# sunwj/SunVolumeRender

Hardware: AMD Instinct MI355X
Metric: Msamples/sec (paths x spp) at 1024^2 on 512^3 volume (higher is better)
Workload: dtype f32; 1 GPU; c3: 512^3 u16 CT-like volume, 1024x1024 image, 3 area lights, env map on, trace depth 1, 256 spp per step; math=bit-exact contract, parallelism=single GPU

## Files before the change

### include/svr_abi.h

```cpp
#ifndef SVR_ABI_H
#define SVR_ABI_H

#include <stddef.h>
#include <stdint.h>

#ifdef __cplusplus
extern "C" {
#endif

#define SVR_MAX_LIGHT_SOURCES 8
#define SVR_TF_TABLE_SIZE 1024

typedef struct svr_vec2 { float x, y; } svr_vec2;
typedef struct svr_vec3 { float x, y, z; } svr_vec3;

typedef struct svr_bbox {
    svr_vec3 vmin, vmax, invSize;
} svr_bbox;

typedef struct svr_volume {
    svr_bbox bbox;
    uint32_t _pad0;
    uint64_t tex;
    float densityScale;
// ... 147 lines not shown
    uint64_t vol_taps;
    uint64_t woodcock_iters;
    uint64_t scatter_events;
    uint64_t shadow_walks;
    uint64_t raycast_steps;
    uint64_t loop_iters;
    uint64_t vol_taps_executed;
    uint64_t walks_ray_skipped;
    uint64_t iters_ray_skipped;
    uint64_t iters_prefix_skipped;
    uint64_t taps_bound_culled;
} svr_counters;
int svr_selftest_chain(const float* items, float* results, uint32_t n);
int svr_selftest_math(int fn, const float* in, uint32_t in_stride, float* out, uint32_t n);
int svr_selftest_bound8(const float* rays, uint32_t n, uint32_t* out);
int svr_macro_grid(int nx, int ny, int nz, int shift_min, int out[8]);
int svr_selftest_accel(int table, void* out, size_t out_bytes, int32_t info[16]);
typedef struct svr_denoise_params {
    int32_t passes;
    float sigma_depth;
    float sigma_normal;
    float sigma_albedo;
    float sigma_opacity;
    float sigma_color;
    float step;
} svr_denoise_params;
int svr_denoise_params_default(svr_denoise_params* p);
int svr_set_denoise_params(const svr_denoise_params* p);
int svr_get_denoise_params(svr_denoise_params* p);
int svr_render_guides(void* guides);
// ... 239 lines not shown
```

### sunvolumerender_amd/abi.py

```python
from __future__ import annotations

import ctypes as C
from pathlib import Path

from ._build import LIB_PATH



class vec2(C.Structure):
    _fields_ = [("x", C.c_float), ("y", C.c_float)]

    def __init__(self, x=0.0, y=0.0):
        super().__init__(float(x), float(y))

    def tuple(self):
        return (self.x, self.y)


class vec3(C.Structure):
    _fields_ = [("x", C.c_float), ("y", C.c_float), ("z", C.c_float)]

    def __init__(self, x=0.0, y=0.0, z=0.0):
        super().__init__(float(x), float(y), float(z))

# ... 313 lines not shown
OPT_LOCAL_MAJORANT = 23
OPT_LIGHT_CULL = 24
OPT_LM_TUNE = 25
OPT_LM_SUBCELLS = 26
OPT_PARK_CHEAP = 27
OPT_PINHOLE_FAST = 28
OPT_POOL = 29
OPT_TRIPS = 30
OPT_NAN_GUARD = 31
OPT_MACRO_SHIFT_MIN = 32
OPT_SPLIT = 33
OPT_ENV_NEE = 34
OPT_FAST_BOUND = 35
OPT_DENOISE_PREVIEW = 36
OPT_NOISE_ESTIMATE = 37
KERNEL_AUTO, KERNEL_PIXEL, KERNEL_TILE, KERNEL_ULOOP, KERNEL_WAVEFRONT = 0, 1, 2, 3, 4

ELEM_I8, ELEM_U8, ELEM_I16, ELEM_U16, ELEM_I32, ELEM_U32, ELEM_F32, ELEM_F64 = range(8)


class MhdHeader(C.Structure):
    _fields_ = [
        ("ndims", C.c_int32), ("dim", C.c_int32 * 3), ("spacing", C.c_double * 3),
        ("elem_type", C.c_int32), ("elem_size", C.c_int32), ("channels", C.c_int32), ("msb", C.c_int32),
        ("compressed", C.c_int32), ("compressed_size", C.c_int64), ("header_size", C.c_int64),
        ("data_offset", C.c_int64), ("data_file", C.c_char * 1024),
    ]


class VolumeInfo(C.Structure):
# ... 35 lines not shown
    "svr_strip_rows_owned": (C.c_uint32, [C.c_uint32, C.c_uint32, C.c_uint32, C.c_uint32]),
    "svr_strip_row_to_y": (C.c_uint32, [C.c_uint32, C.c_uint32, C.c_uint32, C.c_uint32, C.c_uint32]),
    "svr_pack_strips": (C.c_int, [C.c_void_p, C.c_void_p, C.c_uint32, C.c_uint32, C.c_uint32, C.c_uint32, C.c_uint32]),
    "svr_unpack_strips": (C.c_int, [C.c_void_p, C.c_void_p, C.c_uint32, C.c_uint32, C.c_uint32, C.c_uint32, C.c_uint32]),
    "svr_assemble_frame": (C.c_int, [C.c_void_p, C.c_void_p, C.c_void_p, C.c_uint32, C.c_uint32, C.c_uint32, C.c_uint32, C.c_uint32, C.c_uint32]),
    "svr_set_row_shard": (C.c_int, [C.c_uint32, C.c_uint32, C.c_uint32]),
    "svr_set_render_window": (C.c_int, [C.c_int, C.c_int, C.c_int, C.c_int]),
    "svr_set_option": (C.c_int, [C.c_int, C.c_int]),
    "svr_get_option": (C.c_int, [C.c_int]),
    "svr_render_pathtracer_frames": (C.c_int, [C.c_void_p, _P(RenderParams), C.c_uint32]),
    "svr_hdr_to_ldr": (C.c_int, [C.c_void_p, _P(RenderParams)]),
    "svr_hdr_to_ldr_frame": (C.c_int, [C.c_void_p, C.c_void_p, C.c_uint32, C.c_uint32]),
    "svr_selftest_chain": (C.c_int, [C.c_void_p, C.c_void_p, C.c_uint32]),
    "svr_selftest_math": (C.c_int, [C.c_int, C.c_void_p, C.c_uint32, C.c_void_p, C.c_uint32]),
    "svr_selftest_bound8": (C.c_int, [C.c_void_p, C.c_uint32, C.c_void_p]),
    "svr_macro_grid": (C.c_int, [C.c_int, C.c_int, C.c_int, C.c_int, _P(C.c_int)]),
    "svr_selftest_accel": (C.c_int, [C.c_int, C.c_void_p, C.c_size_t, _P(C.c_int32)]),
    "svr_denoise_params_default": (C.c_int, [_P(DenoiseParams)]),
    "svr_set_denoise_params": (C.c_int, [_P(DenoiseParams)]),
    "svr_get_denoise_params": (C.c_int, [_P(DenoiseParams)]),
    "svr_render_guides": (C.c_int, [C.c_void_p]),
    "svr_denoise_to_ldr": (C.c_int, [C.c_void_p, C.c_void_p, C.c_uint32, C.c_uint32, _P(DenoiseParams)]),
    "svr_denoise_hdr": (C.c_int, [C.c_void_p, C.c_void_p, C.c_uint32, C.c_uint32, _P(DenoiseParams)]),
    "svr_guide_builds": (C.c_uint64, []),
    "svr_get_noise_estimate": (C.c_int, [_P(NoiseEstimate), C.c_void_p]),
    "svr_estimate_noise": (C.c_int, [C.c_void_p, C.c_uint32, C.c_void_p, C.c_uint32, C.c_uint32, C.c_uint32, C.c_void_p, _P(NoiseEstimate)]),
    "svr_render_pathtracer_until": (C.c_int, [C.c_void_p, _P(RenderParams), C.c_float, C.c_float, C.c_uint32, _P(C.c_uint32)]),
    "svr_render_pathtracer_adaptive": (C.c_int, [C.c_void_p, _P(RenderParams), C.c_float, C.c_uint32, C.c_uint32, _P(AdaptiveResult)]),
    "svr_get_adaptive_tiles": (C.c_int, [C.c_void_p, C.c_void_p]),
    "svr_projection_params_default": (C.c_int, [_P(ProjectionParams)]),
# ... 101 lines not shown
```

### sunvolumerender_amd/csrc/svr_api.hip

```cpp
#include "../../include/svr_abi.h"
#include "svr_kernels.hpp"
#include "svr_denoise.hpp"
#include "svr_noise.hpp"
#include "svr_project.hpp"
#include "svr_slice.hpp"
#include "svr_hits.hpp"
#include "svr_device.hpp"

#include <hip/hip_runtime.h>
#include <algorithm>
#include <cmath>
#include <cstdarg>
#include <cstdio>
#include <cstdlib>
#include <cstring>
#include <dlfcn.h>
#include <mutex>
#include <string>
#include <unordered_map>
#include <vector>

static_assert(sizeof(svr_vec3) == 12, "glm::vec3 layout");
static_assert(sizeof(svr_bbox) == 36, "cudaBBox layout");
static_assert(sizeof(svr_volume) == 112 && offsetof(svr_volume, tex) == 40 && offsetof(svr_volume, densityScale) == 48 &&
// ... 2401 lines not shown
    case SVR_OPT_QUEUE: return g.opt_queue;
    case SVR_OPT_PARK_END: return g.opt_park_end;
    case SVR_OPT_PARK_CHEAP: return g.opt_park_cheap;
    case SVR_OPT_PINHOLE_FAST: return g.opt_pinhole_fast;
    case SVR_OPT_POOL: return g.opt_pool;
    case SVR_OPT_TRIPS: return g.opt_trips;
    case SVR_OPT_SPLIT: return g.opt_split;
    case SVR_OPT_ENV_NEE: return g.opt_env_nee;
    case SVR_OPT_FAST_BOUND: return g.opt_fast_bound;
    case SVR_OPT_NAN_GUARD: return g.opt_nan_guard;
    case SVR_OPT_MACRO_SHIFT_MIN: return g.opt_macro_shift_min;
    case SVR_OPT_REFILL_MIN_IDLE: return g.opt_refill;
    case SVR_OPT_FRAMES_PER_WAVE_LOG2: return g.opt_frames_log2;
    case SVR_OPT_RAYCAST_LANES_LOG2: return g.opt_rc_lanes;
    case SVR_OPT_FRAME_AHEAD: return g.opt_frame_ahead;
    default: return -1;
    }
}

int svr_selftest_chain(const float* items, float* results, uint32_t n)
{
    if (ensure_init()) return g.err_code;
    if (!items || !results || n == 0) return fail(-4, "svr_selftest_chain: bad arguments");
    float4* d_buf = nullptr;
    HIP_TRY(hipMalloc((void**)&d_buf, (size_t)n * 32));
    hipError_t e = hipMemcpy(d_buf, items, (size_t)n * 16, hipMemcpyHostToDevice);
    if (e == hipSuccess) e = svr::launch_chain_selftest(d_buf, d_buf + n, n, g.stream);
    if (e == hipSuccess) e = hipStreamSynchronize(g.stream);
    if (e == hipSuccess) e = hipMemcpy(results, d_buf + n, (size_t)n * 16, hipMemcpyDeviceToHost);
    hipFree(d_buf);
// ... 25 lines not shown
    if (!g.have_vol || !g.have_tf || !g.have_cam) return fail(-4, "svr_selftest_bound8 before setup_volume/setup_transferfunction/setup_camera");
    svr::DevScene s;
    if (build_scene(g.vol, g.tf, g.cam, s)) return g.err_code;
    if (ensure_mask(s, g.vol, g.tf)) return g.err_code;
    if (s.bnd8 == nullptr) return fail(-3, "svr_selftest_bound8: the fast bound look-up is not in use for this scene");
    float* d_rays = nullptr; uint32_t* d_out = nullptr;
    HIP_TRY(hipMalloc((void**)&d_rays, (size_t)n * 7 * sizeof(float)));
    hipError_t e = hipMalloc((void**)&d_out, (size_t)n * sizeof(uint32_t));
    if (e == hipSuccess) e = hipMemcpy(d_rays, rays, (size_t)n * 7 * sizeof(float), hipMemcpyHostToDevice);
    if (e == hipSuccess) e = svr::launch_bound8_selftest(s, d_rays, n, d_out, g.stream);
    if (e == hipSuccess) e = hipStreamSynchronize(g.stream);
    if (e == hipSuccess) e = hipMemcpy(out, d_out, (size_t)n * sizeof(uint32_t), hipMemcpyDeviceToHost);
    hipFree(d_rays);
    if (d_out) hipFree(d_out);
    if (e != hipSuccess) return fail((int)e, "svr_selftest_bound8 failed: %s", hipGetErrorName(e));
    return 0;
}

int svr_selftest_accel(int table, void* out, size_t out_bytes, int32_t info[16])
{
    if (ensure_init()) return g.err_code;
    if (!info || table < 0 || table > 7 || (table != 0 && !out)) return fail(-4, "svr_selftest_accel: bad arguments");
    if (!g.have_vol || !g.have_tf || !g.have_cam) return fail(-4, "svr_selftest_accel before setup_volume/setup_transferfunction/setup_camera");
    svr::DevScene s;
    if (build_scene(g.vol, g.tf, g.cam, s)) return g.err_code;
    if (ensure_mask(s, g.vol, g.tf)) return g.err_code;
    const Texture* tv = find_tex(g.vol.tex, TEX_VOLUME);
    if (s.empty_mask == nullptr || !tv) return fail(-3, "svr_selftest_accel: the scene has no acceleration data (SVR_OPT_EMPTY_SKIP off?)");
    const int hgx = (tv->mc_gx + 1) / 2, hgy = (tv->mc_gy + 1) / 2, hgz = (tv->mc_gz + 1) / 2;
    const size_t n = (size_t)tv->mc_gx * tv->mc_gy * tv->mc_gz, hn = (size_t)hgx * hgy * hgz;
// ... 71 lines not shown
```

### sunvolumerender_amd/csrc/svr_kernels.hpp

```cpp
#pragma once
#include <hip/hip_runtime.h>
#include <type_traits>
#include "svr_scene.hpp"

namespace svr {

enum { KERNEL_AUTO = 0, KERNEL_PIXEL = 1, KERNEL_TILE = 2, KERNEL_ULOOP = 3, KERNEL_WAVEFRONT = 4, KERNEL_ENV_NEE = 5  };
constexpr int WF_QUEUE_PLANES = 18;
constexpr uint32_t TICKET_SHARDS = 8;
constexpr uint32_t TICKET_STRIDE = 32;
constexpr uint32_t MASK_WORDS_MAX = 8192;
constexpr uint32_t DIST_WORDS_MAX = 4096;
constexpr int DIST_CAP = 15;
constexpr uint32_t REC_C1_WORDS = 17;
constexpr uint32_t REC_A_WORDS = 26;
constexpr uint32_t REC_B_WORDS = 20;
constexpr uint32_t REC_WORDS = REC_A_WORDS + REC_B_WORDS;
constexpr uint32_t QUEUE_TASKS = 32;
constexpr uint32_t QUEUE_CAP = 32 * QUEUE_TASKS;
#ifndef SVR_QUEUE_TASKS_D1
#define SVR_QUEUE_TASKS_D1 64
#endif
#ifndef SVR_QUEUE_CAP_D1
#define SVR_QUEUE_CAP_D1 1024
// ... 72 lines not shown
hipError_t launch_fine_mask(const uint16_t* mm, uint32_t n_cells, const uint32_t* tf_zero_prefix, int tf_n, float densityScale,
                            uint32_t* mask, uint32_t words, hipStream_t stream);
hipError_t launch_sub8(const uint32_t* fine_empty, int fgx, int fgy, int fgz, int gx, int gy, int gz, uint8_t* sub8, hipStream_t stream);
hipError_t launch_bound_class(const uint16_t* mm, int gx, int gy, int gz, const float* tf_rgba, int tf_n, float densityScale,
                              float invSigmaMax, uint32_t* accel, hipStream_t stream);
constexpr uint32_t BOUND8_DIM = 34u;
constexpr uint32_t BOUND8_BYTES = 40960u;
hipError_t launch_bound8(const uint16_t* mm_wide, int hgx, int hgy, int hgz, const float* tf_rgba, int tf_n, float densityScale,
                         float invSigmaMax, uint8_t* bnd8, hipStream_t stream);
hipError_t launch_strips(float* packed, float* frame, uint32_t row_floats, uint32_t n_rows, uint32_t strip_rows, uint32_t rank, uint32_t world,
                         int to_packed, hipStream_t stream);
hipError_t launch_tonemap(const DevScene& scene, const DevWork& work, hipStream_t stream);
hipError_t launch_chain_selftest(const float4* in, float4* out, uint32_t n, hipStream_t stream);
hipError_t launch_math_selftest(int fn, const float* in, uint32_t in_stride, float* out, uint32_t n, hipStream_t stream);
hipError_t launch_bound8_selftest(const DevScene& scene, const float* rays, uint32_t n, uint32_t* out, hipStream_t stream);
hipError_t launch_raycast(const DevScene& scene, const DevWork& work, float stepSize, bool count, int num_cus, int lanes_log2, hipStream_t stream);
hipError_t launch_repack(const uint16_t* src, uint16_t* dst, int nx, int ny, int nz, int layout,
                         int sy, int sz, int bnx, int bny, hipStream_t stream);

}
```

### sunvolumerender_amd/csrc/svr_lanes.hpp

```cpp
#pragma once
#include "svr_walk.hpp"
#include "svr_tile_tasks.hpp"

namespace svr {


enum { PH_PRIMARY = 0, PH_REFILL, PH_SHADE, PH_CHEAP, PH_FETCH, PH_MARCH, PH_END, PH_FOLD, PH_N };
enum { PH_TICKET = PH_N + 1, PH_LOOP, PH_FIRST, PH_END_ALL };
enum { PROF_SHADOW_WALKS = 2 * PH_END_ALL, PROF_RECORDS };
constexpr uint32_t PROF_WORDS = 2 * PH_END_ALL + 2;
#ifdef SVR_TEST_HOOKS
#define SVR_PROF 1
struct ProfScope {
    unsigned long long* acc; uint32_t ph; uint64_t t0;
    __device__ ProfScope(unsigned long long* a, uint32_t p) : acc(a), ph(p), t0(__builtin_amdgcn_s_memtime()) {}
    __device__ void end(uint32_t lanes)
    {
        const uint64_t dt = __builtin_amdgcn_s_memtime() - t0;
        if ((threadIdx.x & 63u) == 0u) { atomicAdd(&acc[2 * ph], (unsigned long long)dt); atomicAdd(&acc[2 * ph + 1], (unsigned long long)dt * lanes); }
    }
};
#define PROF_BEGIN(name, ph) ProfScope name(c_prof, ph)
#define PROF_END(name, lanes) name.end(lanes)
#else
#define SVR_PROF 0
// ... 647 lines not shown
```

### sunvolumerender_amd/csrc/svr_primary.hpp

```cpp
#pragma once
#include "svr_walk.hpp"
#include "svr_lanes.hpp"

namespace svr {

#ifndef SVR_SHADOW_REMARCH
#define SVR_SHADOW_REMARCH true
#endif
#ifndef SVR_PRIMARY_REMARCH
#define SVR_PRIMARY_REMARCH false
#endif

template <int LAYOUT, bool COUNT, bool SKIP, typename LDS>
SVR_DEV bool trace_primary(const DevScene& s, const LDS& L_, uint32_t x, uint32_t y, uint32_t hashed, bool group_march, uint32_t P2,
                           GroupMapShared* gslot, Cnt& c, Rng& rng, v3& L, v3& pt, v3& wo, float& val, const DevScene* scp = nullptr)
{
    const DevScene& sc = scp ? *scp : s;
    uint32_t offset = y * sc.imageW + x;
    rng_init(rng, hashed + offset);
    if (COUNT) c.paths++;
    L = V3(0.f, 0.f, 0.f);
    const v3 T = V3(1.f, 1.f, 1.f);
    v3 orig, dir;
    camera_ray(sc, x, y, rng, orig, dir);
    float ls_t;
    int ls_id = nearest_light(sc, orig, dir, ls_t);
    float tMin = (float)1e-6, tMax = SVR_FLT_MAX;
    val = 0.f;
    float t;
    if (SKIP && group_march) {
        float t_occ;
        GroupMap map;
        map.g = gslot + ((threadIdx.x & 63u) & ((1u << P2) - 1u) & (GROUP_MAPS_PER_WAVE - 1u));
        int r = walk_setup_group<COUNT, SKIP>(s, L_, P2, orig, dir, false, tMin, tMax, t_occ, map);
        t = r <= 0 ? -SVR_FLT_MAX
                   : walk_run<LAYOUT, COUNT, SKIP, false, true>(s, L_, orig, dir, rng, tMin, tMax, t_occ, val, false, c, &map, P2);
    } else
        t = walk<LAYOUT, COUNT, SKIP, SVR_PRIMARY_REMARCH>(s, L_, orig, dir, rng, tMin, tMax, val, false, c);
    if (ls_id >= 0) {
        float tt = t < 0.f ? SVR_FLT_MAX : t;
        if (ls_t < tt) {
            const DevLight& l = sc.lights[ls_id];
            float cosTerm = dot(V3(l.normal[0], l.normal[1], l.normal[2]), -dir);
            L = L + (T * V3(l.radiance[0], l.radiance[1], l.radiance[2])) * (cosTerm <= 0.f ? 0.f : 1.f);
            return false;
        }
    }
    if (t < 0.f) {
        if (sc.env_on_escape) L = L + T * env_radiance(sc, dir);
// ... 40 lines not shown
```

### sunvolumerender_amd/csrc/svr_selftest.hip

```cpp
#include "svr_kernels.hpp"
#include "svr_device.hpp"
#include "svr_walk.hpp"
#include "svr_chain.hpp"

namespace svr {

__global__ __launch_bounds__(256) void k_math_selftest(int fn, const float* __restrict__ in, uint32_t stride, float* __restrict__ out, uint32_t n)
{
    const uint32_t i = blockIdx.x * 256u + threadIdx.x;
    if (i >= n) return;
    const float* a = in + (size_t)i * stride;
    const float x = a[0], y = stride > 1 ? a[1] : 0.f, z = stride > 2 ? a[2] : 0.f;
    float r = 0.f, sn, cs;
    switch (fn) {
    case 0: r = schlick_fresnel(x, y, z); break;
    case 1: r = logf_(x); break;
    case 2: r = expf_(x); break;
    case 3: sincosf_(x, &sn, &cs); r = sn; break;
    case 4: sincosf_(x, &sn, &cs); r = cs; break;
    case 5: r = acosf_(x); break;
    case 6: r = atan2f_(x, y); break;
    case 7: r = powf_(x, y); break;
    case 8: {
        Rng g;
// ... 43 lines not shown
}

hipError_t launch_bound8_selftest(const DevScene& s, const float* rays, uint32_t n, uint32_t* out, hipStream_t st)
{
    const dim3 grid((n + 255u) / 256u), block(256);
    switch (s.layout) {
    case 1: hipLaunchKernelGGL(k_bound8_selftest<1>, grid, block, 0, st, s, rays, n, out); break;
    case 2: hipLaunchKernelGGL(k_bound8_selftest<2>, grid, block, 0, st, s, rays, n, out); break;
    case 3: hipLaunchKernelGGL(k_bound8_selftest<3>, grid, block, 0, st, s, rays, n, out); break;
    case 4: hipLaunchKernelGGL(k_bound8_selftest<4>, grid, block, 0, st, s, rays, n, out); break;
    default: return hipErrorInvalidValue;
    }
    return hipGetLastError();
}

__global__ void k_chain_selftest(const float4* __restrict__ in, float4* __restrict__ out, uint32_t n_items)
{
    uint32_t i = blockIdx.x * blockDim.x + threadIdx.x;
    if (i >= n_items) return;
    const float4 q = in[i];
    bool e0, e1, ok;
    const uint32_t c0 = chain_count(q.x, q.y, q.z, false, e0);
    const uint32_t c1 = chain_count(q.x, q.y, q.z, true, e1);
    const float ta = chain_advance(q.x, q.y, (uint32_t)q.w, ok);
    out[i] = make_float4(__uint_as_float(c0), __uint_as_float(c1), ta, __uint_as_float((e0 ? 1u : 0u) | (e1 ? 2u : 0u) | (ok ? 4u : 0u)));
}

hipError_t launch_chain_selftest(const float4* in, float4* out, uint32_t n, hipStream_t st)
{
    hipLaunchKernelGGL(k_chain_selftest, dim3((n + 255u) / 256u), dim3(256), 0, st, in, out, n);
// ... 5 lines not shown
```

### sunvolumerender_amd/csrc/svr_trace_tile.hip

```cpp
#include "svr_walk.hpp"
#include "svr_lanes.hpp"
#include "svr_tile_tasks.hpp"
#include "svr_primary.hpp"

namespace svr {

#ifdef SVR_TEST_HOOKS
#define SVR_DEBUG_STOPS 1
#else
#define SVR_DEBUG_STOPS 0
#endif

#ifndef SVR_SHADOW_REMARCH
#define SVR_SHADOW_REMARCH true
#endif
#ifndef SVR_PRIMARY_REMARCH
#define SVR_PRIMARY_REMARCH false
#endif

template <int LAYOUT, bool COUNT, bool SKIP, bool DEPTH1, typename LDS>
SVR_DEV v3 trace_path_tile(const DevScene& s, const LDS& L_, uint32_t x, uint32_t y, uint32_t traceDepth_,
                           uint32_t hashed, uint32_t debug_stop, bool group_march, uint32_t P2, GroupMapShared* gslot, Cnt& c)
{
    const uint32_t traceDepth = DEPTH1 ? 1u : traceDepth_;
// ... 144 lines not shown
    const uint32_t wave = threadIdx.x >> 6;
#ifndef SVR_COLD_SCENE
#define SVR_COLD_SCENE 1
#endif
    auto cold_scene = [&]() -> const DevScene* {
        if constexpr (QUEUE && (DEPTH1 || (POOL && SVR_COLD_DEEP_POOL) || SVR_COLD_DEEP_ALL) && SVR_COLD_SCENE) {
            auto p = __builtin_amdgcn_kernarg_segment_ptr();
            asm volatile("" : "+s"(p));
            return (const DevScene*)p;
        } else return nullptr;
    };
    const TaskShape ts = task_shape(w);
    const uint32_t fl2 = ts.fl2, P2 = ts.P2, tw2 = ts.tw2, th2 = ts.th2, wv = ts.wv, fgroups = ts.fgroups;
    const uint32_t n_tasks = ts.n_tasks;
    Cnt c = {0, 0, 0, 0, 0, 0, 0, 0, 0, 0};

    const uint32_t unit = w.unit;
    const uint32_t n_units = (n_tasks + unit - 1u) / unit;
    const uint32_t shard0 = blockIdx.x % TICKET_SHARDS;
    const bool fold = w.fold != 0u;
    uint32_t npend = 0, qC = 0, qA = 0, qB = 0;
    LaneQueue Q;
    Q.cap = DRAIN_CAP;
    Q.q = QUEUE ? w.queue + (size_t)(blockIdx.x * TILE_WAVES + wave) * (REC_WORDS * DRAIN_CAP) : nullptr;
    float* const gpend = QUEUE ? w.pend + (size_t)(blockIdx.x * TILE_WAVES + wave) * (DRAIN_TASKS * 3u * 64u) : nullptr;
    auto flush = [&]() {
        if constexpr (QUEUE) {
            __builtin_amdgcn_fence(__ATOMIC_RELEASE, "workgroup");
            __builtin_amdgcn_fence(__ATOMIC_ACQUIRE, "workgroup");
            if constexpr (POOL && !DEPTH1) {
// ... 128 lines not shown
                    Rng rng = {0u, 0u, 0u, 0u, 0u, 0u};
                    v3 L = V3(0.f, 0.f, 0.f);
                    bool hit = false;
                    float val = 0.f;
                    Shade vs;
                    vs.pt = L; vs.wo = L; vs.gradient = L; vs.color[0] = vs.color[1] = vs.color[2] = vs.color[3] = 0.f; vs.Pbrdf = 0.f; vs.st = 0;
                    Nee ne;
                    ne.wi = L; ne.B = L; ne.pdf = 1.f; ne.light = 0u; ne.have = false;
#if SVR_PROF
                    unsigned long long* c_prof = w.counters + CNT_N;
#endif
                    PROF_BEGIN(pa, PH_PRIMARY);
#if SVR_PROF
                    const uint32_t prof_i0 = c.iters - c.iskip;
#endif
                    if (live) {
                        uint32_t x = w.x0 + px, y = owned_row_to_y(w, r);
                        hit = trace_primary<LAYOUT, COUNT, SKIP>(s, lds, x, y, wang_hash(w.frame0 + slot), group_march, P2, &gmaps[wave][0], c, rng, L, vs.pt, vs.wo, val, cold_scene());
                    }
                    PROF_END(pa, (uint32_t)__popcll(__ballot(live)));
#if SVR_PROF
                    if (COUNT && DEPTH1) {
                        const uint32_t d = (c.iters - c.iskip) - prof_i0;
                        uint32_t m = d;
                        for (int o = 32; o > 0; o >>= 1) m = max(m, (uint32_t)__shfl_xor((int)m, o));
                        const unsigned long long sum = wave_sum(d);
                        if (lane == 0) { atomicAdd(&c_prof[2 * PH_N], (unsigned long long)m * 64ull); atomicAdd(&c_prof[2 * PH_N + 1], sum); }
                    }
#endif
                    const bool shade_here = DEPTH1 || !s.bound_cull;
                    {
                        const uint64_t mh = __ballot(hit);
                        if (shade_here && mh != 0ull) {
                            PROF_BEGIN(psh, PH_SHADE);
// ... 99 lines not shown
    PROF_END(ploop, 64u);
    if (COUNT) cnt_flush(w, c);
}

template <int LAYOUT, bool COUNT>
static hipError_t launch_tile_t(const DevScene& s, const DevWork& w, const LaunchCfg& cfg, hipStream_t st)
{
    uint32_t wv = w.x1 - w.x0;
    if (wv == 0 || w.n_rows == 0) return hipSuccess;
    if (w.fold && w.nframes > 64u) return hipErrorInvalidValue;
    DevWork w2;
    TaskGrid g;
    hipError_t e = task_launch_setup(w, cfg, SVR_TILE_THREADS / 64, w.fold != 0u, cfg.frames_log2, st, w2, g);
    if (e != hipSuccess) return e;
    const uint32_t blocks = g.blocks;
    if (cfg.unit_override > 0) w2.unit = (uint32_t)cfg.unit_override;
    const bool skip = s.empty_mask != nullptr, d1 = w.traceDepth == 1u;
    const bool queue = LAYOUT != LAYOUT_LINEAR && w.queue != nullptr && w.pend != nullptr && blocks <= w.queue_blocks && w.traceDepth < 32768u &&
                       (w.fold || !COUNT);
#define SVR_LAUNCH_TILE(SK, D1, QU) hipLaunchKernelGGL((k_trace_tile<LAYOUT, COUNT, SK, D1, QU>), dim3(blocks), dim3(SVR_TILE_THREADS), 0, st, s, w2)
    if constexpr (LAYOUT != LAYOUT_LINEAR && !COUNT) {
        if (queue && !w.fold) {
#define SVR_LAUNCH_DIRECT(SK, D1, PO) hipLaunchKernelGGL((k_trace_tile<LAYOUT, false, SK, D1, true, PO, true>), dim3(blocks), dim3(SVR_TILE_THREADS), 0, st, s, w2)
            if (skip && cfg.pool_primary) { if (d1) SVR_LAUNCH_DIRECT(true, true, true); else SVR_LAUNCH_DIRECT(true, false, true); }
            else if (skip && d1) SVR_LAUNCH_DIRECT(true, true, false);
            else if (skip) SVR_LAUNCH_DIRECT(true, false, false);
            else if (d1) SVR_LAUNCH_DIRECT(false, true, false);
            else SVR_LAUNCH_DIRECT(false, false, false);
#undef SVR_LAUNCH_DIRECT
            return hipGetLastError();
        }
    }
    if constexpr (LAYOUT != LAYOUT_LINEAR) {
        if (queue && skip && cfg.pool_primary) {
// ... 29 lines not shown
```

### sunvolumerender_amd/csrc/svr_walk.hpp

```cpp
#pragma once
#include "svr_kernel_common.hpp"
#include <type_traits>

namespace svr {

struct LdsTile {
    float alpha[SVR_TF_MAX + SVR_TF_PAD];
    uint32_t dist[DIST_WORDS_MAX];
    uint32_t mask[MASK_WORDS_MAX];
    uint32_t emask[MASK_WORDS_MAX];
};
struct LdsTileNoMask {
    float alpha[SVR_TF_MAX + SVR_TF_PAD];
    uint32_t dist[1];
    uint32_t mask[1];
    uint32_t emask[1];
};
struct LdsTileCull : LdsTile {
    uint32_t cls[DIST_WORDS_MAX];
    float thr[BOUND_CLASSES];
};
struct LdsBound8 {
    uint8_t bnd[BOUND8_BYTES];
};
// ... 244 lines not shown
    struct { float lo, dt, inv_dt; const uint64_t* w; } g = {gm.lo, gm.dt, gm.inv_dt, gm.g->w};
    const uint32_t fl2 = 6u - P2, Lg = 64u >> P2;
    int ki = (int)((t - g.lo) * g.inv_dt) - 1;
    const uint32_t k = (uint32_t)(ki < 0 ? 0 : ki);
    const uint32_t r = k >> fl2, j = k & (Lg - 1u);
    uint64_t w0 = r == 0u ? g.w[0] : (r == 1u ? g.w[1] : (r == 2u ? g.w[2] : 0ull));
    w0 >>= (j << P2);
    if (w0) return fma_((float)(k + ((uint32_t)__builtin_ctzll(w0) >> P2)), g.dt, g.lo);
    const uint64_t w1 = r == 0u ? g.w[1] : (r == 1u ? g.w[2] : 0ull);
    if (w1) return fma_((float)(((r + 1u) << fl2) + ((uint32_t)__builtin_ctzll(w1) >> P2)), g.dt, g.lo);
    const uint64_t w2 = r == 0u ? g.w[2] : 0ull;
    if (w2) return fma_((float)(((r + 2u) << fl2) + ((uint32_t)__builtin_ctzll(w2) >> P2)), g.dt, g.lo);
    return u2f(SVR_INF_BITS);
}

template <typename LDS>
SVR_DEV float first_occupied_group(const DevScene& s, const LDS& L, uint32_t P2, v3 o, v3 d, bool hit, float tMin, float tMax, bool& ok,
                                   GroupMap& map)
{
    GroupMapShared& ms = *map.g;
    map.valid = false; map.lo = 0.f; map.dt = 1.f; map.inv_dt = 1.f;
    for (uint32_t r = 0; r < GROUP_MAP_ROUNDS; ++r) ms.w[r] = 0ull;
    const float INF = u2f(SVR_INF_BITS);
    const uint32_t lane = threadIdx.x & 63u;
    const uint32_t pl = lane & ((1u << P2) - 1u), m = lane >> P2, Lg = 64u >> P2;
    const int leader = (int)pl;
    const v3 oc = V3(__shfl(o.x, leader, 64), __shfl(o.y, leader, 64), __shfl(o.z, leader, 64));
    const v3 dc = V3(__shfl(d.x, leader, 64), __shfl(d.y, leader, 64), __shfl(d.z, leader, 64));
    float lo = hit ? tMin : INF, hi = hit ? tMax : -INF;
    for (uint32_t off = 32u; off >= (1u << P2); off >>= 1) {
// ... 24 lines not shown
        const int iz = min(max((int)__builtin_floorf(fma_(Bz, tk, Az)), 0), gz - 1);
        const uint32_t q = (uint32_t)(ix + iy * gx + iz * s.mc_gxy);
        const bool occupied = (tk <= hi) && !((L.mask[q >> 5] >> (q & 31u)) & 1u);
        const uint64_t b = __ballot(occupied) & gmask;
        if (round < GROUP_MAP_ROUNDS) ms.w[round] = b >> pl;
        if (b && !found) { found = true; result = fma_((float)(k0 + (((uint32_t)__builtin_ctzll(b) - pl) >> P2)), dt, lo); }
        const bool at_end = fma_((float)(k0 + Lg - 1u), dt, lo) > hi;
        if (at_end) { complete = round < GROUP_MAP_ROUNDS; break; }
        if (found && round + 1u >= GROUP_MAP_ROUNDS) break;
    }
    map.lo = lo; map.dt = dt; map.inv_dt = bmax * (1.f / 0.7f);
    map.valid = complete && ok;
    __builtin_amdgcn_fence(__ATOMIC_RELEASE, "wavefront");
    __builtin_amdgcn_fence(__ATOMIC_ACQUIRE, "wavefront");
    return result;
}

template <bool COUNT, bool SKIP, typename LDS>
SVR_DEV int walk_setup(const DevScene& s, const LDS& L, v3 orig, v3 dir, bool rng_live, float& tMin, float& tMax, float& t_occ)
{
    float tNear, tFar;
    if (!volume_intersect(s, orig, dir, tNear, tFar)) return -1;
    tMin = tNear < 0.f ? (float)1e-6 : tNear;
    tMax = tFar;
    t_occ = tMin;
    if (SKIP && s.ray_skip) {
        t_occ = first_occupied(s, L, orig, dir, tMin, tMax);
        if (!COUNT && !rng_live && t_occ == u2f(SVR_INF_BITS)) return 0;
    }
    return 1;
// ... 134 lines not shown
```

Baseline: 10720 Msamples/s.

## Share wave-wide empty-space march across 2x1 pixel blocks for pinhole primaries

Adds a shared group march for pinhole primary rays. A wave marches the macro-cell occupancy grid once along a central ray and keeps the result in LDS, tagged by a 2x1 pixel block and frame group. A later wave-step on the same block reuses it when every lane's ray passes an admission test (same origin, small angular deviation, interval contained). The launch sets the work unit to the march block size so consecutive tasks hit the same block. The aim is to halve the occupancy-grid marching cost per primary ray. Rays that fail admission fall back to a per-ray first_occupied walk, and there is added LDS state and branching. A selftest entry point is also added.

```diff
diff --git a/include/svr_abi.h b/include/svr_abi.h
--- a/include/svr_abi.h
+++ b/include/svr_abi.h
@@ -185,6 +185,7 @@
 int svr_selftest_chain(const float* items, float* results, uint32_t n);
 int svr_selftest_math(int fn, const float* in, uint32_t in_stride, float* out, uint32_t n);
 int svr_selftest_bound8(const float* rays, uint32_t n, uint32_t* out);
+int svr_selftest_group_march(uint32_t frame0, uint64_t out[8]);
 int svr_macro_grid(int nx, int ny, int nz, int shift_min, int out[8]);
 int svr_selftest_accel(int table, void* out, size_t out_bytes, int32_t info[16]);
 typedef struct svr_denoise_params {
diff --git a/sunvolumerender_amd/abi.py b/sunvolumerender_amd/abi.py
--- a/sunvolumerender_amd/abi.py
+++ b/sunvolumerender_amd/abi.py
@@ -351,6 +351,7 @@
 OPT_FAST_BOUND = 35
 OPT_DENOISE_PREVIEW = 36
 OPT_NOISE_ESTIMATE = 37
+OPT_UNIT = 101
 KERNEL_AUTO, KERNEL_PIXEL, KERNEL_TILE, KERNEL_ULOOP, KERNEL_WAVEFRONT = 0, 1, 2, 3, 4
 
 ELEM_I8, ELEM_U8, ELEM_I16, ELEM_U16, ELEM_I32, ELEM_U32, ELEM_F32, ELEM_F64 = range(8)
@@ -416,6 +417,7 @@
     "svr_selftest_chain": (C.c_int, [C.c_void_p, C.c_void_p, C.c_uint32]),
     "svr_selftest_math": (C.c_int, [C.c_int, C.c_void_p, C.c_uint32, C.c_void_p, C.c_uint32]),
     "svr_selftest_bound8": (C.c_int, [C.c_void_p, C.c_uint32, C.c_void_p]),
+    "svr_selftest_group_march": (C.c_int, [C.c_uint32, C.c_void_p]),
     "svr_macro_grid": (C.c_int, [C.c_int, C.c_int, C.c_int, C.c_int, _P(C.c_int)]),
     "svr_selftest_accel": (C.c_int, [C.c_int, C.c_void_p, C.c_size_t, _P(C.c_int32)]),
     "svr_denoise_params_default": (C.c_int, [_P(DenoiseParams)]),
diff --git a/sunvolumerender_amd/csrc/svr_api.hip b/sunvolumerender_amd/csrc/svr_api.hip
--- a/sunvolumerender_amd/csrc/svr_api.hip
+++ b/sunvolumerender_amd/csrc/svr_api.hip
@@ -2439,6 +2439,7 @@
     case SVR_OPT_FRAMES_PER_WAVE_LOG2: return g.opt_frames_log2;
     case SVR_OPT_RAYCAST_LANES_LOG2: return g.opt_rc_lanes;
     case SVR_OPT_FRAME_AHEAD: return g.opt_frame_ahead;
+    case 101: return g.opt_unit;
     default: return -1;
     }
 }
@@ -2494,6 +2495,26 @@
     hipFree(d_rays);
     if (d_out) hipFree(d_out);
     if (e != hipSuccess) return fail((int)e, "svr_selftest_bound8 failed: %s", hipGetErrorName(e));
+    return 0;
+}
+
+int svr_selftest_group_march(uint32_t frame0, uint64_t out[8])
+{
+    if (ensure_init()) return g.err_code;
+    if (!out) return fail(-4, "svr_selftest_group_march: bad arguments");
+    if (!g.have_vol || !g.have_tf || !g.have_cam) return fail(-4, "svr_selftest_group_march before setup_volume/setup_transferfunction/setup_camera");
+    svr::DevScene s;
+    if (build_scene(g.vol, g.tf, g.cam, s)) return g.err_code;
+    if (ensure_mask(s, g.vol, g.tf)) return g.err_code;
+    if (s.empty_mask == nullptr || !s.ray_skip) return fail(-3, "svr_selftest_group_march: the scene has no whole-ray test (SVR_OPT_EMPTY_SKIP off, or a clip box beyond the volume)");
+    unsigned long long* d_out = nullptr;
+    HIP_TRY(hipMalloc((void**)&d_out, 8 * sizeof(unsigned long long)));
+    hipError_t e = hipMemsetAsync(d_out, 0, 8 * sizeof(unsigned long long), g.stream);
+    if (e == hipSuccess) e = svr::launch_group_march_selftest(s, frame0, d_out, g.stream);
+    if (e == hipSuccess) e = hipStreamSynchronize(g.stream);
+    if (e == hipSuccess) e = hipMemcpy(out, d_out, 8 * sizeof(unsigned long long), hipMemcpyDeviceToHost);
+    hipFree(d_out);
+    if (e != hipSuccess) return fail((int)e, "svr_selftest_group_march failed: %s", hipGetErrorName(e));
     return 0;
 }
 
diff --git a/sunvolumerender_amd/csrc/svr_kernels.hpp b/sunvolumerender_amd/csrc/svr_kernels.hpp
--- a/sunvolumerender_amd/csrc/svr_kernels.hpp
+++ b/sunvolumerender_amd/csrc/svr_kernels.hpp
@@ -110,6 +110,7 @@
 hipError_t launch_chain_selftest(const float4* in, float4* out, uint32_t n, hipStream_t stream);
 hipError_t launch_math_selftest(int fn, const float* in, uint32_t in_stride, float* out, uint32_t n, hipStream_t stream);
 hipError_t launch_bound8_selftest(const DevScene& scene, const float* rays, uint32_t n, uint32_t* out, hipStream_t stream);
+hipError_t launch_group_march_selftest(const DevScene& scene, uint32_t frame0, unsigned long long* out, hipStream_t stream);
 hipError_t launch_raycast(const DevScene& scene, const DevWork& work, float stepSize, bool count, int num_cus, int lanes_log2, hipStream_t stream);
 hipError_t launch_repack(const uint16_t* src, uint16_t* dst, int nx, int ny, int nz, int layout,
                          int sy, int sz, int bnx, int bny, hipStream_t stream);
diff --git a/sunvolumerender_amd/csrc/svr_lanes.hpp b/sunvolumerender_amd/csrc/svr_lanes.hpp
--- a/sunvolumerender_amd/csrc/svr_lanes.hpp
+++ b/sunvolumerender_amd/csrc/svr_lanes.hpp
@@ -7,8 +7,9 @@
 
 enum { PH_PRIMARY = 0, PH_REFILL, PH_SHADE, PH_CHEAP, PH_FETCH, PH_MARCH, PH_END, PH_FOLD, PH_N };
 enum { PH_TICKET = PH_N + 1, PH_LOOP, PH_FIRST, PH_END_ALL };
-enum { PROF_SHADOW_WALKS = 2 * PH_END_ALL, PROF_RECORDS };
-constexpr uint32_t PROF_WORDS = 2 * PH_END_ALL + 2;
+enum { PROF_SHADOW_WALKS = 2 * PH_END_ALL, PROF_RECORDS, PROF_MARCH };
+constexpr uint32_t PROF_WORDS = 2 * PH_END_ALL + 6;
+static_assert(PROF_WORDS <= 32u, "the debug words behind the counters (svr_api.hip, DEBUG_WORDS)");
 #ifdef SVR_TEST_HOOKS
 #define SVR_PROF 1
 struct ProfScope {
diff --git a/sunvolumerender_amd/csrc/svr_primary.hpp b/sunvolumerender_amd/csrc/svr_primary.hpp
--- a/sunvolumerender_amd/csrc/svr_primary.hpp
+++ b/sunvolumerender_amd/csrc/svr_primary.hpp
@@ -11,9 +11,10 @@
 #define SVR_PRIMARY_REMARCH false
 #endif
 
-template <int LAYOUT, bool COUNT, bool SKIP, typename LDS>
+template <int LAYOUT, bool COUNT, bool SKIP, bool SHARE = false, typename LDS>
 SVR_DEV bool trace_primary(const DevScene& s, const LDS& L_, uint32_t x, uint32_t y, uint32_t hashed, bool group_march, uint32_t P2,
-                           GroupMapShared* gslot, Cnt& c, Rng& rng, v3& L, v3& pt, v3& wo, float& val, const DevScene* scp = nullptr)
+                           GroupMapShared* gslot, Cnt& c, Rng& rng, v3& L, v3& pt, v3& wo, float& val, const DevScene* scp = nullptr, uint32_t fg = 0u,
+                           uint32_t* march_did = nullptr)
 {
     const DevScene& sc = scp ? *scp : s;
     uint32_t offset = y * sc.imageW + x;
@@ -32,7 +33,13 @@
         float t_occ;
         GroupMap map;
         map.g = gslot + ((threadIdx.x & 63u) & ((1u << P2) - 1u) & (GROUP_MAPS_PER_WAVE - 1u));
-        int r = walk_setup_group<COUNT, SKIP>(s, L_, P2, orig, dir, false, tMin, tMax, t_occ, map);
+        int r;
+        bool shared = false;
+        if constexpr (SHARE && SVR_MARCH_BLOCK > 1) shared = P2 == 0u && sc.cam_pinhole != 0u;
+        if (shared)
+            r = walk_setup_shared<COUNT, SKIP>(s, sc, L_, x, y, fg, orig, dir, false, tMin, tMax, t_occ, gslot, map, march_did);
+        else
+            r = walk_setup_group<COUNT, SKIP>(s, L_, P2, orig, dir, false, tMin, tMax, t_occ, map);
         t = r <= 0 ? -SVR_FLT_MAX
                    : walk_run<LAYOUT, COUNT, SKIP, false, true>(s, L_, orig, dir, rng, tMin, tMax, t_occ, val, false, c, &map, P2);
     } else
diff --git a/sunvolumerender_amd/csrc/svr_selftest.hip b/sunvolumerender_amd/csrc/svr_selftest.hip
--- a/sunvolumerender_amd/csrc/svr_selftest.hip
+++ b/sunvolumerender_amd/csrc/svr_selftest.hip
@@ -81,6 +81,62 @@
     return hipGetLastError();
 }
 
+__global__ __launch_bounds__(256) void k_group_march_selftest(const DevScene s, uint32_t frame0, unsigned long long* __restrict__ out)
+{
+    __shared__ LdsTileCull lds;
+    __shared__ GroupMapShared gmaps[4][GROUP_MAPS_PER_WAVE];
+    lds_tile_load(lds, s, true);
+    const uint32_t lane = threadIdx.x & 63u, wave = threadIdx.x >> 6;
+    GroupMapShared* gslot = &gmaps[wave][0];
+    march_kept_reset(gslot);
+    unsigned long long n_bad = 0, n_pts = 0, n_hit = 0, n_valid = 0, n_did[5] = {0, 0, 0, 0, 0};
+    const uint32_t hashed = wang_hash(frame0 + lane);
+    for (uint32_t y = blockIdx.x * 4u + wave; y < s.imageH; y += gridDim.x * 4u) {
+        for (uint32_t x = 0; x < s.imageW; ++x) {
+            Rng rng;
+            rng_init(rng, hashed + (y * s.imageW + x));
+            v3 orig, dir;
+            camera_ray(s, x, y, rng, orig, dir);
+            float tMin, tMax, t_occ;
+            GroupMap map;
+            uint32_t did = MARCH_NONE;
+            const int r = walk_setup_shared<true, true>(s, s, lds, x, y, 0u, orig, dir, false, tMin, tMax, t_occ, gslot, map, &did);
+            n_did[did]++;
+            const float bmax = fmax_(__builtin_fabsf(dir.x * s.mc_scale[0]), fmax_(__builtin_fabsf(dir.y * s.mc_scale[1]), __builtin_fabsf(dir.z * s.mc_scale[2])));
+            if (r >= 0) { n_hit++; if (map.valid) n_valid++; }
+            const float dtc = 0.125f / bmax;
+            float clear_until = t_occ;
+            for (uint32_t i = 0; i < 65536u && r >= 0 && bmax > 0.f; ++i) {
+                const float t = fma_((float)i, dtc, tMin);
+                if (t > tMax) break;
+                if (t >= clear_until && map.valid) {
+                    const float nx = group_map_next(map, 0u, t);
+                    if (nx > t) clear_until = nx;
+                    continue;
+                }
+                if (t >= clear_until) continue;
+                const Cell c = cell_of(s, orig + dir * t);
+                const uint32_t ux = (uint32_t)(c.cx + 1), uy = (uint32_t)(c.cy + 1), uz = (uint32_t)(c.cz + 1);
+                if (!((ux <= (uint32_t)s.nx) & (uy <= (uint32_t)s.ny) & (uz <= (uint32_t)s.nz))) continue;
+                n_pts++;
+                if (!cell_is_empty<false>(lds, s, c)) n_bad++;
+            }
+        }
+    }
+    const unsigned long long tot[4] = {wave_sum(n_bad), wave_sum(n_pts), wave_sum(n_hit), wave_sum(n_valid)};
+    if (lane == 0) {
+        atomicAdd(&out[0], tot[0]); atomicAdd(&out[1], tot[1]); atomicAdd(&out[6], tot[2]); atomicAdd(&out[7], tot[3]);
+        for (uint32_t k = 1; k < 5u; ++k) atomicAdd(&out[1 + k], n_did[k]);
+    }
+}
+
+hipError_t launch_group_march_selftest(const DevScene& s, uint32_t frame0, unsigned long long* out, hipStream_t st)
+{
+    const uint32_t blocks = (s.imageH + 3u) / 4u;
+    hipLaunchKernelGGL(k_group_march_selftest, dim3(blocks < 1024u ? blocks : 1024u), dim3(256), 0, st, s, frame0, out);
+    return hipGetLastError();
+}
+
 __global__ void k_chain_selftest(const float4* __restrict__ in, float4* __restrict__ out, uint32_t n_items)
 {
     uint32_t i = blockIdx.x * blockDim.x + threadIdx.x;
diff --git a/sunvolumerender_amd/csrc/svr_trace_tile.hip b/sunvolumerender_amd/csrc/svr_trace_tile.hip
--- a/sunvolumerender_amd/csrc/svr_trace_tile.hip
+++ b/sunvolumerender_amd/csrc/svr_trace_tile.hip
@@ -182,6 +182,8 @@
     const uint32_t fl2 = ts.fl2, P2 = ts.P2, tw2 = ts.tw2, th2 = ts.th2, wv = ts.wv, fgroups = ts.fgroups;
     const uint32_t n_tasks = ts.n_tasks;
     Cnt c = {0, 0, 0, 0, 0, 0, 0, 0, 0, 0};
+    constexpr bool SHARE = Drain::WIDE && !SVR_TILE_LIST && SVR_MARCH_BLOCK > 1;
+    if constexpr (SHARE) march_kept_reset(&gmaps[wave][0]);
 
     const uint32_t unit = w.unit;
     const uint32_t n_units = (n_tasks + unit - 1u) / unit;
@@ -340,10 +342,15 @@
 #if SVR_PROF
                     const uint32_t prof_i0 = c.iters - c.iskip;
 #endif
+                    uint32_t march_did = MARCH_NONE;
                     if (live) {
                         uint32_t x = w.x0 + px, y = owned_row_to_y(w, r);
-                        hit = trace_primary<LAYOUT, COUNT, SKIP>(s, lds, x, y, wang_hash(w.frame0 + slot), group_march, P2, &gmaps[wave][0], c, rng, L, vs.pt, vs.wo, val, cold_scene());
-                    }
+                        hit = trace_primary<LAYOUT, COUNT, SKIP, SHARE>(s, lds, x, y, wang_hash(w.frame0 + slot), group_march, P2, &gmaps[wave][0], c, rng, L, vs.pt, vs.wo, val, cold_scene(), fg,
+                                                                              SVR_PROF ? &march_did : nullptr);
+                    }
+#if SVR_PROF
+                    if (lane == 0 && march_did != MARCH_NONE) atomicAdd(&c_prof[PROF_MARCH + march_did - 1u], 1ull);
+#endif
                     PROF_END(pa, (uint32_t)__popcll(__ballot(live)));
 #if SVR_PROF
                     if (COUNT && DEPTH1) {
@@ -473,10 +480,12 @@
     hipError_t e = task_launch_setup(w, cfg, SVR_TILE_THREADS / 64, w.fold != 0u, cfg.frames_log2, st, w2, g);
     if (e != hipSuccess) return e;
     const uint32_t blocks = g.blocks;
-    if (cfg.unit_override > 0) w2.unit = (uint32_t)cfg.unit_override;
     const bool skip = s.empty_mask != nullptr, d1 = w.traceDepth == 1u;
     const bool queue = LAYOUT != LAYOUT_LINEAR && w.queue != nullptr && w.pend != nullptr && blocks <= w.queue_blocks && w.traceDepth < 32768u &&
                        (w.fold || !COUNT);
+    if (SVR_MARCH_BLOCK > 1 && !SVR_TILE_LIST && queue && skip && d1 && !cfg.pool_primary && w2.frames_log2 == 6u && w.nframes <= 64u && s.cam_pinhole && s.ray_skip)
+        w2.unit = SVR_MARCH_BLOCK;
+    if (cfg.unit_override > 0) w2.unit = (uint32_t)cfg.unit_override;
 #define SVR_LAUNCH_TILE(SK, D1, QU) hipLaunchKernelGGL((k_trace_tile<LAYOUT, COUNT, SK, D1, QU>), dim3(blocks), dim3(SVR_TILE_THREADS), 0, st, s, w2)
     if constexpr (LAYOUT != LAYOUT_LINEAR && !COUNT) {
         if (queue && !w.fold) {
diff --git a/sunvolumerender_amd/csrc/svr_walk.hpp b/sunvolumerender_amd/csrc/svr_walk.hpp
--- a/sunvolumerender_amd/csrc/svr_walk.hpp
+++ b/sunvolumerender_amd/csrc/svr_walk.hpp
@@ -282,6 +282,47 @@
     return u2f(SVR_INF_BITS);
 }
 
+SVR_DEV bool group_admit(const DevScene& s, v3 o, v3 d, v3 oc, v3 dc, float hi)
+{
+    const float dev = fmax_(__builtin_fabsf((d.x - dc.x) * s.mc_scale[0]),
+                            fmax_(__builtin_fabsf((d.y - dc.y) * s.mc_scale[1]), __builtin_fabsf((d.z - dc.z) * s.mc_scale[2])));
+    return (o.x == oc.x) && (o.y == oc.y) && (o.z == oc.z) && (dev * hi <= 0.25f);
+}
+
+template <typename LDS>
+SVR_DEV bool group_march_ray(const DevScene& s, const LDS& L, v3 oc, v3 dc, float lo, float hi, GroupMap& map, float& result, bool& complete)
+{
+    GroupMapShared& ms = *map.g;
+    const float INF = u2f(SVR_INF_BITS);
+    const uint32_t lane = threadIdx.x & 63u;
+    result = INF; complete = false;
+    const float Ax = fma_(oc.x - s.vmin[0], s.mc_scale[0], s.mc_off), Bx = dc.x * s.mc_scale[0];
+    const float Ay = fma_(oc.y - s.vmin[1], s.mc_scale[1], s.mc_off), By = dc.y * s.mc_scale[1];
+    const float Az = fma_(oc.z - s.vmin[2], s.mc_scale[2], s.mc_off), Bz = dc.z * s.mc_scale[2];
+    const float bmax = fmax_(__builtin_fabsf(Bx), fmax_(__builtin_fabsf(By), __builtin_fabsf(Bz)));
+    if (!(bmax > 0.f)) return false;
+    const float dt = 0.7f / bmax;
+    const int gx = s.mc_gx, gy = s.mc_gy, gz = s.mc_gz;
+    bool found = false;
+    uint32_t round = 0;
+    for (uint32_t k0 = 0u; k0 < 4096u; k0 += 64u, ++round) {
+        const float tk = fma_((float)(k0 + lane), dt, lo);
+        const int ix = min(max((int)__builtin_floorf(fma_(Bx, tk, Ax)), 0), gx - 1);
+        const int iy = min(max((int)__builtin_floorf(fma_(By, tk, Ay)), 0), gy - 1);
+        const int iz = min(max((int)__builtin_floorf(fma_(Bz, tk, Az)), 0), gz - 1);
+        const uint32_t q = (uint32_t)(ix + iy * gx + iz * s.mc_gxy);
+        const bool occupied = (tk <= hi) && !((L.mask[q >> 5] >> (q & 31u)) & 1u);
+        const uint64_t b = __ballot(occupied);
+        if (round < GROUP_MAP_ROUNDS) ms.w[round] = b;
+        if (b && !found) { found = true; result = fma_((float)(k0 + (uint32_t)__builtin_ctzll(b)), dt, lo); }
+        const bool at_end = fma_((float)(k0 + 63u), dt, lo) > hi;
+        if (at_end) { complete = round < GROUP_MAP_ROUNDS; break; }
+        if (found && round + 1u >= GROUP_MAP_ROUNDS) break;
+    }
+    map.lo = lo; map.dt = dt; map.inv_dt = bmax * (1.f / 0.7f);
+    return true;
+}
+
 template <typename LDS>
 SVR_DEV float first_occupied_group(const DevScene& s, const LDS& L, uint32_t P2, v3 o, v3 d, bool hit, float tMin, float tMax, bool& ok,
                                    GroupMap& map)
@@ -336,6 +377,111 @@
     __builtin_amdgcn_fence(__ATOMIC_RELEASE, "wavefront");
     __builtin_amdgcn_fence(__ATOMIC_ACQUIRE, "wavefront");
     return result;
+}
+
+#ifndef SVR_MARCH_BLOCK
+#define SVR_MARCH_BLOCK 2
+#endif
+static_assert(SVR_MARCH_BLOCK == 1 || SVR_MARCH_BLOCK == 2, "march blocks: 1 (every pixel marches) or 2 (2 x 1 pixels)");
+template <bool MAX>
+SVR_DEV float wave_minmax(float v)
+{
+    for (int off = 32; off > 0; off >>= 1) { const float o = __shfl_xor(v, off, 64); v = MAX ? fmax_(v, o) : fmin_(v, o); }
+    return v;
+}
+
+struct MarchKept {
+    enum { TAG = 0, RESULT, LO, HI, DT, INV_DT, OX, OY, OZ, DX, DY, DZ, COMPLETE, WORDS };
+};
+static_assert(MarchKept::WORDS * 4u <= 2u * sizeof(GroupMapShared) && GROUP_MAPS_PER_WAVE >= 3u, "the kept march fits into slots 1 and 2");
+constexpr uint32_t MARCH_TAG_NONE = 0xffffffffu;
+SVR_DEV uint32_t march_tag(uint32_t x, uint32_t y, uint32_t fg) { return (((y << 15) ^ (x >> 1)) + fg * 0x9e3779b1u) & 0x7fffffffu; }
+SVR_DEV void march_kept_reset(GroupMapShared* gslot)
+{
+    reinterpret_cast<uint32_t*>(gslot + 1)[MarchKept::TAG] = MARCH_TAG_NONE;
+    __builtin_amdgcn_fence(__ATOMIC_RELEASE, "wavefront");
+    __builtin_amdgcn_fence(__ATOMIC_ACQUIRE, "wavefront");
+}
+
+enum MarchDid : uint32_t { MARCH_NONE = 0, MARCH_SHARED, MARCH_REUSED, MARCH_REFUSED, MARCH_ALONE };
+
+template <bool COUNT, bool SKIP, typename LDS>
+SVR_DEV int walk_setup_shared(const DevScene& s, const DevScene& sc, const LDS& L, uint32_t x, uint32_t y, uint32_t fg, v3 orig, v3 dir, bool rng_live,
+                              float& tMin, float& tMax, float& t_occ, GroupMapShared* gslot, GroupMap& map, uint32_t* did = nullptr)
+{
+    map.g = gslot;
+    map.valid = false; map.lo = 0.f; map.dt = 1.f; map.inv_dt = 1.f;
+    float tNear, tFar;
+    const bool hit = volume_intersect(s, orig, dir, tNear, tFar);
+    tMin = tNear < 0.f ? (float)1e-6 : tNear;
+    tMax = tFar;
+    t_occ = tMin;
+    if (did) *did = MARCH_NONE;
+    if (!(SKIP && s.ray_skip)) return hit ? 1 : -1;
+    if (__ballot(hit) == 0ull) return -1;
+    const float INF = u2f(SVR_INF_BITS);
+    uint32_t* kw = reinterpret_cast<uint32_t*>(gslot + 1);
+    const uint32_t tag = march_tag(x, y, fg);
+    float g = INF;
+    bool ok = false, complete = false, have = false;
+    if (kw[MarchKept::TAG] == tag) {
+        const v3 oc = V3(u2f(kw[MarchKept::OX]), u2f(kw[MarchKept::OY]), u2f(kw[MarchKept::OZ]));
+        const v3 dc = V3(u2f(kw[MarchKept::DX]), u2f(kw[MarchKept::DY]), u2f(kw[MarchKept::DZ]));
+        const float lo = u2f(kw[MarchKept::LO]), hi = u2f(kw[MarchKept::HI]);
+        ok = group_admit(s, orig, dir, oc, dc, hi) && tMin >= lo && tMax <= hi;
+        if (__ballot(hit && !ok) == 0ull) {
+            have = true;
+            g = u2f(kw[MarchKept::RESULT]);
+            complete = kw[MarchKept::COMPLETE] != 0u;
+            map.lo = lo; map.dt = u2f(kw[MarchKept::DT]); map.inv_dt = u2f(kw[MarchKept::INV_DT]);
+            if (did) *did = MARCH_REUSED;
+        } else if (did) *did = MARCH_REFUSED;
+    }
+    if (!have) {
+        const bool fresh = kw[MarchKept::TAG] != tag;
+        float lo = wave_minmax<false>(hit ? tMin : INF), hi = wave_minmax<true>(hit ? tMax : -INF);
+        v3 oc = V3(u2f((uint32_t)__builtin_amdgcn_readfirstlane((int)f2u(orig.x))), u2f((uint32_t)__builtin_amdgcn_readfirstlane((int)f2u(orig.y))),
+                   u2f((uint32_t)__builtin_amdgcn_readfirstlane((int)f2u(orig.z))));
+        v3 dc = V3(0.f, 0.f, 0.f);
+        bool shared = false;
+        if (fresh) {
+            float nx = 2.f * ((float)(x | 1u) / sc.wm1) - 1.f, ny = 2.f * (((float)y + 0.5f) / sc.hm1) - 1.f;
+            nx = nx * sc.aspectRatio * sc.tanFovxOverTwo * sc.focalLength;
+            ny = ny * sc.tanFovxOverTwo * sc.focalLength;
+            const v3 v = (V3(sc.cam_u[0], sc.cam_u[1], sc.cam_u[2]) * nx + V3(sc.cam_v[0], sc.cam_v[1], sc.cam_v[2]) * ny) -
+                         V3(sc.cam_w[0], sc.cam_w[1], sc.cam_w[2]) * sc.focalLength;
+            dc = v * __builtin_amdgcn_rsqf(dot(v, v));
+            const float bmax = fmax_(__builtin_fabsf(dc.x * s.mc_scale[0]), fmax_(__builtin_fabsf(dc.y * s.mc_scale[1]), __builtin_fabsf(dc.z * s.mc_scale[2])));
+            const float dt = 0.7f / bmax;
+            const float lo_w = lo - dt, hi_w = hi + dt;
+            ok = group_admit(s, orig, dir, oc, dc, hi_w);
+            shared = __ballot(hit && !ok) == 0ull;
+            if (shared) { lo = lo_w; hi = hi_w; }
+        }
+        if (!shared) {
+            dc = V3(u2f((uint32_t)__builtin_amdgcn_readfirstlane((int)f2u(dir.x))), u2f((uint32_t)__builtin_amdgcn_readfirstlane((int)f2u(dir.y))),
+                    u2f((uint32_t)__builtin_amdgcn_readfirstlane((int)f2u(dir.z))));
+            ok = group_admit(s, orig, dir, oc, dc, hi);
+        }
+        if (did && *did == MARCH_NONE) *did = shared ? MARCH_SHARED : MARCH_ALONE;
+        for (uint32_t r = 0; r < GROUP_MAP_ROUNDS; ++r) gslot->w[r] = 0ull;
+        const bool marched = group_march_ray(s, L, oc, dc, lo, hi, map, g, complete);
+        if (!marched) { ok = false; g = INF; }
+        kw[MarchKept::TAG] = marched ? tag : MARCH_TAG_NONE;
+        kw[MarchKept::RESULT] = f2u(g); kw[MarchKept::LO] = f2u(lo); kw[MarchKept::HI] = f2u(hi);
+        kw[MarchKept::DT] = f2u(map.dt); kw[MarchKept::INV_DT] = f2u(map.inv_dt);
+        kw[MarchKept::OX] = f2u(oc.x); kw[MarchKept::OY] = f2u(oc.y); kw[MarchKept::OZ] = f2u(oc.z);
+        kw[MarchKept::DX] = f2u(dc.x); kw[MarchKept::DY] = f2u(dc.y); kw[MarchKept::DZ] = f2u(dc.z);
+        kw[MarchKept::COMPLETE] = complete ? 1u : 0u;
+        __builtin_amdgcn_fence(__ATOMIC_RELEASE, "wavefront");
+        __builtin_amdgcn_fence(__ATOMIC_ACQUIRE, "wavefront");
+    }
+    map.valid = complete && ok;
+    if (hit) {
+        t_occ = ok ? g : first_occupied(s, L, orig, dir, tMin, tMax);
+        if (!COUNT && !rng_live && t_occ == u2f(SVR_INF_BITS)) return 0;
+    }
+    return hit ? 1 : -1;
 }
 
 template <bool COUNT, bool SKIP, typename LDS>
```

After: 10920 Msamples/s, median of 6. 1.9% higher.
